# nackdai/aten

Measured on AMD Instinct MI355X. Metric: Mrays/sec (W*H*spp/1e6/s, reference definition), Sponza 1080p 1spp 5-bounce, higher is better.
Workload: dtype f32; 1 GPU; sponza_lod 1920x1080 1spp 5-bounce GGX+IBL, reference-built sponza_lod.sbvh (stand-in for missing sponza.obj); width=1920, height=1080, spp=1, max_depth=5, rr_depth=3, frames_in_flight=4, triangles=12852, bvh_nodes=38000, anyhit_twins=1, planar_area_lights=0

## Files before the change

### aten_amd/_hostlib.py

```python
import ctypes as C
import os

from . import build

_lib = None

ATNS_ABI_VERSION = 2

ORDER_AS_SPLIT, ORDER_AREA, ORDER_AREA_SMALL, ORDER_COUNT, ORDER_COUNT_SMALL, ORDER_NEAR_POINT = range(6)


class BvhOptions(C.Structure):
    _fields_ = [("spatial_splits", C.c_int32), ("spatial_alpha", C.c_float), ("object_bins", C.c_int32),
                ("spatial_bins", C.c_int32), ("sweep_below", C.c_int32), ("child_order", C.c_int32),
                ("max_refs_factor", C.c_float), ("order_point", C.c_float * 3),
                ("order_point_given", C.c_int32), ("reinsert_iterations", C.c_int32), ("reinsert_batch", C.c_float)]


class BvhStats(C.Structure):
    _fields_ = [("n_nodes", C.c_uint32), ("n_leaves", C.c_uint32), ("n_spatial_splits", C.c_uint32), ("n_reinsertions", C.c_uint32),
                ("sah_cost", C.c_float)]


def default_bvh_options(**kw):
# ... 32 lines not shown
                                            C.POINTER(BvhStats)]
        lib.atns_optimize_nodes.restype = C.c_int
        lib.atns_anyhit_twin.argtypes = [C.c_void_p, C.c_uint32, C.POINTER(C.c_void_p), C.POINTER(C.c_double), C.POINTER(C.c_double)]
        lib.atns_anyhit_twin.restype = C.c_int
        lib.atns_build_blas.argtypes = [C.c_void_p, C.c_void_p, C.c_void_p, C.c_uint32,
                                        C.POINTER(C.c_void_p), C.POINTER(C.c_uint32),
                                        C.POINTER(C.c_float), C.POINTER(C.c_float)]
        lib.atns_build_blas.restype = C.c_int
        lib.atns_build_tlas.argtypes = [C.c_void_p, C.c_void_p, C.c_void_p, C.c_void_p, C.c_uint32,
                                        C.POINTER(C.c_void_p), C.POINTER(C.c_uint32)]
        lib.atns_build_tlas.restype = C.c_int
        lib.atns_free.argtypes = [C.c_void_p]
        lib.atns_free.restype = None
        lib.atns_validate_nodes.argtypes = [C.c_void_p, C.c_uint32]
        lib.atns_validate_nodes.restype = C.c_int64
        lib.atns_create_camera.argtypes = [C.c_void_p, C.POINTER(C.c_float), C.POINTER(C.c_float), C.POINTER(C.c_float),
                                           C.c_float, C.c_float, C.c_float, C.c_int32, C.c_int32]
        lib.atns_create_camera.restype = C.c_int
        _lib = lib
    return _lib
```

### aten_amd/_lib.py

```python
import ctypes as C
import os

from . import build

_lib = None

K_NAMES = ["gen_path", "trace_closest", "shade", "trace_shadow", "accumulate_sample", "gather",
           "svgf_prepare", "svgf_temporal", "svgf_variance", "svgf_atrous", "trace_fused"]

SYMBOLS = [
    "atn_create", "atn_destroy", "atn_last_error", "atn_upload_scene", "atn_update_camera", "atn_update_tlas",
    "atn_init_sampler", "atn_set_random", "atn_set_screen_shard", "atn_render", "atn_reset", "atn_set_path_batches",
    "atn_set_frames_in_flight", "atn_bank_streams", "atn_side_stream", "atn_mgpu_set_frames_in_flight", "atn_set_sampling_options", "atn_sample_texture",
    "atn_svgf_render", "atn_svgf_set_motion_depth", "atn_svgf_reset", "atn_svgf_set_atrous_iterations",
    "atn_svgf_download", "atn_svgf_output_device", "atn_svgf_set_dilate_temporal_weight", "atn_svgf_denoise", "atn_svgf_upload",
    "atn_restir_set_options", "atn_restir_render", "atn_restir_set_motion_depth", "atn_restir_reset", "atn_restir_capture",
    "atn_restir_download", "atn_npr_render", "atn_npr_reset", "atn_npr_capture", "atn_npr_download",
    "atn_volume_render", "atn_volume_reset", "atn_volume_capture", "atn_volume_download", "atn_volume_phase_table",
    "atn_film_device", "atn_tile_device", "atn_tile_slots", "atn_anyhit_twins", "atn_planar_area_lights", "atn_stream", "atn_synchronize",
    "atn_assemble_tiles", "atn_assemble_tiles_on", "atn_download_film", "atn_upload_film", "atn_get_stats", "atn_get_kernel_times",
    "atn_reset_kernel_times", "atn_generate_paths", "atn_trace_closest", "atn_cmj_samples", "atn_cmj_batch", "atn_ray_offset", "atn_get_random", "atn_random_count",
    "atn_material_table", "atn_material_eval", "atn_compact", "atn_compact2", "atn_sizeof_scene_desc", "atn_sizeof_destination",
    "atn_abi_version", "atn_build_id",
    "atn_download_path_cost", "atn_update_geometry", "atn_scene_device_arrays", "atn_lbvh_rebuild_list", "atn_lbvh_build",
    "atn_mgpu_update_geometry", "atn_mgpu_lbvh_rebuild_list",
    "atn_skin_create", "atn_skin_update", "atn_skin_compute", "atn_lbvh_rebuild_list_skinned", "atn_skin_download",
    "atn_skin_download_list", "atn_skin_destroy",
    "atn_mgpu_create", "atn_mgpu_destroy", "atn_mgpu_last_error", "atn_mgpu_shard_count", "atn_mgpu_shard_device",
    "atn_mgpu_upload_scene", "atn_mgpu_update_tlas", "atn_mgpu_update_camera", "atn_mgpu_init_sampler",
    "atn_mgpu_set_random", "atn_mgpu_render", "atn_mgpu_reset", "atn_mgpu_synchronize", "atn_mgpu_film_device",
    "atn_mgpu_download_film",
    "atn_set_regeneration", "atn_get_regeneration", "atn_render_burst", "atn_regen_stage_counts",
    "atn_mgpu_set_regeneration", "atn_mgpu_render_burst", "atn_set_upload_options", "atn_libm_probe", "atn_set_shade_math",
]
# ... 72 lines not shown
        l.atn_npr_download.argtypes = [vp, C.c_int32, vp]
        l.atn_volume_render.argtypes = [vp, vp, vp]
        l.atn_volume_reset.argtypes = [vp]
        l.atn_volume_capture.argtypes = [vp, C.c_int32]
        l.atn_volume_download.argtypes = [vp, C.c_int32, vp]
        l.atn_volume_phase_table.argtypes = [vp, C.c_float, C.c_uint32, vp, vp, vp, vp, vp, vp]
        l.atn_svgf_set_dilate_temporal_weight.argtypes = [vp, C.c_int32]
        l.atn_svgf_denoise.argtypes = [vp, vp, C.c_int32, vp, vp]
        l.atn_svgf_upload.argtypes = [vp, C.c_int32, C.c_int32, C.c_int32, vp]
        l.atn_svgf_output_device.argtypes = [vp]
        l.atn_svgf_output_device.restype = vp
        l.atn_film_device.argtypes = [vp]; l.atn_film_device.restype = vp
        l.atn_tile_device.argtypes = [vp]; l.atn_tile_device.restype = vp
        l.atn_tile_slots.argtypes = [vp]; l.atn_tile_slots.restype = C.c_uint32
        l.atn_anyhit_twins.argtypes = [vp]; l.atn_anyhit_twins.restype = C.c_uint32
        l.atn_planar_area_lights.argtypes = [vp]; l.atn_planar_area_lights.restype = C.c_uint32
        l.atn_stream.argtypes = [vp]; l.atn_stream.restype = vp
        l.atn_side_stream.argtypes = [vp]; l.atn_side_stream.restype = vp
        l.atn_synchronize.argtypes = [vp]
        l.atn_assemble_tiles.argtypes = [vp, vp, C.c_int32, vp]
        l.atn_assemble_tiles_on.argtypes = [vp, vp, C.c_int32, vp, vp]
        l.atn_download_film.argtypes = [vp, vp]
        l.atn_upload_film.argtypes = [vp, C.c_int32, C.c_int32, vp]
        l.atn_get_stats.argtypes = [vp, vp]
        l.atn_get_kernel_times.argtypes = [vp, vp, vp]
        l.atn_reset_kernel_times.argtypes = [vp]
        l.atn_generate_paths.argtypes = [vp, C.c_int32, C.c_int32, C.c_int32, C.c_uint32, vp]
        l.atn_trace_closest.argtypes = [vp, vp, C.c_uint32, C.c_float, C.c_float, vp, vp]
        l.atn_cmj_samples.argtypes = [vp, C.c_uint32, C.c_uint32, C.c_uint32, C.c_int32, vp]
        l.atn_cmj_batch.argtypes = [vp, C.c_uint32, vp, vp, vp, C.c_int32, vp]
# ... 29 lines not shown
```

### aten_amd/csrc/aten_amd.hip

```cpp
#include <hip/hip_runtime.h>

#include <algorithm>
#include <cstdio>
#include <cstdlib>
#include <chrono>
#include <cstring>
#include <memory>
#include <random>
#include <string>
#include <vector>

#include "../../include/aten_amd.h"
#include "device/kernels.hpp"
#include "device/launch.hpp"
#include "device/svgf.hpp"
#include "device/restir.hpp"
#include "device/npr.hpp"
#include "device/volume.hpp"
#include "device/lbvh.hpp"
#include "device/skinning.hpp"
#include "host/scene_upload.hpp"
#include "host/ibl_precompute.hpp"

namespace atn {
// ... 74 lines not shown

    DevBuf<float4> nodes, vtx_pos, vtx_nml, matrices, texels, carpaint, shade_tris;
    DevBuf<atn_triangle_param> tris;
    DevBuf<atn_object_param> objects;
    DevBuf<DevMaterial> materials;
    DevBuf<atn_light_param> lights;
    DevBuf<float4> light_plane;
    DevBuf<DevTexture> textures;
    DevBuf<atn_toon_param> toon;
    DevBuf<atn_light_param> npr_lights;
    DevBuf<float> screen_shadow;
    DevBuf<uint32_t> texels8;
    DevScene scene{};
    bool has_scene = false, has_camera = false;
    std::vector<int32_t> list_root_link;
    uint32_t n_planar_lights = 0;
    struct PlanarCert {
        int32_t inst_obj = -1, mesh_obj = -1, mtx_id = -1;
        atn_object_param inst{}, mesh{};
        atn_mat4 l2w{}, w2l{};
        uint32_t tri_first = 0, tri_count = 0, vtx_lo = 0, vtx_hi = 0;
    };
    std::vector<PlanarCert> planar_certs;
    void collect_planar_certs(const atn_scene_desc* s, const std::vector<atn_light_param>& lights)
    {
        planar_certs.clear();
        for (size_t i = 0; i < lights.size() && i < s->n_lights; i++) {
            if (!lights[i]._pad) continue;
            PlanarCert c;
            c.inst_obj = s->lights[i].arealight_objid;
// ... 529 lines not shown
        { const int vrc = vol_decode(s, img); if (vrc) return vrc; }
        env_host.clear(); env_w = env_h = 0; ibl_tables_ready = false;
        {
            const int32_t ei = s->config.bg.envmap_tex_idx;
            if (ei >= 0 && (uint32_t)ei < s->n_textures && s->config.bg.enable_env_map) {
                const atn_texture_desc& t = s->textures[ei];
                env_host.assign(t.texels, t.texels + (size_t)t.width * t.height);
                env_w = t.width; env_h = t.height; env_multiplyer = s->config.bg.multiplyer;
            }
        }
        {
            int orc = apply_sampling_options();
            if (orc) return orc;
        }
        list_root_link = img.list_root_link; list_twin_delta = img.list_twin_delta; tlas_refs = img.tlas_refs;
        list_base = img.list_root; list_bytes = img.list_bytes; list_tri_leaves = img.list_tri_leaves; list_inner = img.list_inner;
        n_scene_tris = s->n_triangles; n_scene_vtx = s->n_vertices; n_scene_mtrls = s->n_materials;
        top_base = img.list_root[0];
        n_bottom_nodes = img.n_nodes - s->bvh_lists[0].count;
        n_host_matrices = s->n_matrices;
        host_matrices.assign(s->matrices, s->matrices + s->n_matrices);
        tree_is_deep = img.n_nodes >= kRefillMinNodes;
        return ATN_OK;
    }

    int apply_sampling_options()
    {
        scene.tex_bilinear = opt_tex_bilinear;
        scene.ibl_importance = 0;
        scene.ibl_cdf_v = nullptr; scene.ibl_cdf_u = nullptr; scene.ibl_w = 0; scene.ibl_h = 0;
// ... 232 lines not shown
        if ((uint64_t)tri_offset + n > n_scene_tris) return fail(ATN_ERR_INVALID_ARG, "triangle range outside the uploaded scene");
        if (list_tri_leaves[list] != n || list_inner[list] != n - 1 || list_bytes[list] != (n - 1) * kInnerBytes + n * kTriLeafBytes)
            return fail(ATN_ERR_UNSUPPORTED, "the list was not uploaded as a binary tree with one leaf per triangle of this range");
        ATN_HIP(hipSetDevice(device));
        const int32_t twin_word = list < list_twin_delta.size() ? list_twin_delta[list] : 0;
        const uint32_t twin_delta = (uint32_t)(twin_word & ~15), twin_dirs = twin_word == 0 ? 0u : ((twin_word & 1) ? 8u : 1u);
        if (twin_word != 0 && twin_delta != list_bytes[list]) return fail(ATN_ERR_UNSUPPORTED, "the list's twins do not lie at the list's own size apart");
        { int r = begin_scene_update(64); if (r) return r; }
        if (!box_dev) { int r = repack_shade_tris(tri_offset, n); if (r) return r; }
        { int r = lbvh_enqueue(tris.p + tri_offset, n, (int32_t)tri_offset, bmin, bmax, vtx_pos.p, 0, list_base[list], upd, box_dev); if (r) return r; }
        const uint32_t nn = 2 * n - 1;
        hipLaunchKernelGGL(k_lbvh_emit, dim3((nn + 255) / 256), dim3(256), 0, upd, n, (const atn_bvh_node*)lb.ref_nodes.p, (const uint32_t*)lb.offs.p,
                           (const atn_triangle_param*)tris.p, (const float4*)vtx_pos.p, nodes.p);
        ATN_HIP(hipGetLastError());
        log_range(SB_NODES, list_base[list], list_bytes[list]);
        if (twin_dirs) {
            if (lb.flips.n < n) ATN_HIP(lb.flips.resize(n));
            LbvhTopo t{ lb.left.p, lb.right.p, lb.parent.p, lb.first.p, lb.last.p };
            hipLaunchKernelGGL(k_lbvh_twin_flips, dim3((n + 255) / 256), dim3(256), 0, upd, n, t, (const atn_bvh_node*)lb.ref_nodes.p, twin_dirs, lb.flips.p);
            hipLaunchKernelGGL(k_lbvh_twin_emit, dim3((nn + 255) / 256, twin_dirs), dim3(256), 0, upd, n, t, (const atn_bvh_node*)lb.ref_nodes.p,
                               (const uint32_t*)lb.offs.p, (const uint8_t*)lb.flips.p, twin_delta, (const atn_triangle_param*)tris.p, (const float4*)vtx_pos.p, nodes.p);
            ATN_HIP(hipGetLastError());
            log_range(SB_NODES, list_base[list] + twin_delta, (size_t)twin_dirs * twin_delta);
        }
        { int r = end_scene_update(); if (r) return r; }
        if (sync) ATN_HIP(hipStreamSynchronize(upd));
        return ATN_OK;
    }

    struct Skin {
// ... 288 lines not shown
    {
        uint32_t b = (n + 255u) / 256u;
        if (b == 0) b = 1;
        return b < cap_blocks ? b : cap_blocks;
    }

    bool tree_is_deep = false;
    static constexpr size_t kRefillMinNodes = 2048;
    static constexpr uint32_t kRefillMinPaths = 400u * 1000u;
    bool refill_walk(bool frame) const
    {
        if (env_flavour >= 0) return env_flavour == 1;
        return tree_is_deep && (!frame || n_slots >= kRefillMinPaths);
    }

    uint32_t lds_scene_bytes() const
    {
        const uint64_t b = (uint64_t)scene.node_bytes + (uint64_t)scene.mtx_quads * 16u;
        return (env_lds_nodes && b <= kLdsNodesMaxBytes) ? (uint32_t)b : 0u;
    }

    uint32_t trace_grid(uint32_t n_jobs, bool refill) const
    {
        if (refill) {
            const uint32_t waves_per_block = (uint32_t)kTraceBlock / 64u;
            uint32_t blocks = ((n_jobs + atn::kFetchChunk - 1u) / atn::kFetchChunk + waves_per_block - 1u) / waves_per_block;
            if (blocks < 1u) blocks = 1u;
            const uint32_t cap = (frames_in_flight > 1 ? 256u * 18u : 256u * 32u) / waves_per_block;
            return blocks < cap ? blocks : cap;
        }
// ... 94 lines not shown
        for (int k = 0; k < nb; k++) {
            const uint32_t begin = (uint32_t)k * per;
            const uint32_t end = begin + per < n_slots ? begin + per : n_slots;
            if (begin >= end) continue;
            hipStream_t st = nb > 1 ? bstream[k] : stream;
            if (nb > 1) ATN_HIP(hipStreamWaitEvent(st, ev_fork, 0));
            PathBuffers pb = buffers(count, k, begin);
            fp.slot_begin = (int32_t)begin; fp.slot_end = (int32_t)end;
            const uint32_t n = end - begin;
            const PassPlan plan = plan_pass(SVGF ? PassKind::Svgf : PassKind::Serial, n);
            fp.chunk_items = plan.shade_items;
            const uint32_t g_slots = grid_for(n), g_all = (n + 255u) / 256u;
            for (int32_t s = 0; s < d->sample; s++) {
                fp.sample = s;
                if (s > 0) ATN_HIP(hipMemsetAsync(pb.q_count, 0, (size_t)4 * counters_depth * 4, st));
                prof_begin(prof, ATN_K_GEN, st);
                hipLaunchKernelGGL(k_gen_path, dim3(g_slots), dim3(256), 0, st, pb, fp, camera, (const uint32_t*)seeds.p);
                prof_end(prof);
                if (count || !fuse_traces) {
                    for (int32_t b = 0; b < d->maxDepth; b++) {
                        prof_begin(prof, ATN_K_TRACE_CLOSEST, st);
                        launch_trace<false>(plan, pb, count, b, st);
                        prof_end(prof);
                        prof_begin(prof, ATN_K_SHADE, st);
                        launch_shade<SVGF>(plan, st, pb, fp, b, sv);
                        prof_end(prof);
                        prof_begin(prof, ATN_K_TRACE_SHADOW, st);
                        launch_trace<true>(plan, pb, count, b, st);
                        prof_end(prof);
                    }
                }
                else {
                    for (int32_t b = 0; b <= d->maxDepth; b++) {
                        const TraceLaunch tl = trace_launch(plan, b);
                        prof_begin(prof, tl.prof_kind, st);
                        launch_trace_fused<false>(tl, st, pb, scene, b - 1, b < d->maxDepth ? b : -1, b);
                        prof_end(prof);
                        if (b < d->maxDepth) {
                            prof_begin(prof, ATN_K_SHADE, st);
                            launch_shade<SVGF>(plan, st, pb, fp, b, sv);
                            prof_end(prof);
                        }
                    }
                }
                if (SVGF || d->sample > 1) {
                    prof_begin(prof, ATN_K_ACCUM, st);
                    if (SVGF) hipLaunchKernelGGL(k_svgf_sample_end, dim3(g_all), dim3(256), 0, st, pb, fp, sf);
                    else hipLaunchKernelGGL(k_accumulate_sample, dim3(g_all), dim3(256), 0, st, pb, fp);
                    prof_end(prof);
                }
            }
            if (nb > 1) {
// ... 1399 lines not shown
    if (which == 9) { r.sv_motion_set = true; r.sv_motion_count = (size_t)width * height; }
    return ATN_OK;
}
void* atn_svgf_output_device(atn_ctx* ctx) { return ctx ? (void*)ctx->r.sv_out.p : nullptr; }

void* atn_film_device(atn_ctx* ctx) { return ctx ? (void*)ctx->r.film.p : nullptr; }
void* atn_tile_device(atn_ctx* ctx) { return ctx ? (void*)ctx->r.tile_out.p : nullptr; }
uint32_t atn_tile_slots(atn_ctx* ctx) { return ctx ? ctx->r.n_slots : 0; }
uint32_t atn_planar_area_lights(atn_ctx* ctx) { return (ctx && ctx->r.scene.planar_lights) ? ctx->r.n_planar_lights : 0u; }
uint32_t atn_anyhit_twins(atn_ctx* ctx)
{
    uint32_t n = 0;
    if (ctx) for (const int32_t d : ctx->r.list_twin_delta) n += d != 0 ? 1u : 0u;
    return n;
}
void* atn_stream(atn_ctx* ctx) { return ctx ? (void*)ctx->r.stream : nullptr; }
void* atn_side_stream(atn_ctx* ctx)
{
    if (!ctx) return nullptr;
    try { if (ctx->r.quiesce() != ATN_OK) return nullptr; return (void*)ctx->r.get_side_stream(); } catch (...) { return nullptr; }
}

int atn_synchronize(atn_ctx* ctx)
{
    CTX_QUIET_OR_FAIL(ctx);
    C_HIP(ctx->r, hipStreamSynchronize(ctx->r.stream));
    return ATN_OK;
}

int atn_assemble_tiles(atn_ctx* ctx, const void* gathered_dev, int32_t world, void* film_dev_out)
// ... 429 lines not shown
```

### aten_amd/csrc/device/kernels.hpp

```cpp
#pragma once
#include "shading.hpp"
#include "toon.hpp"

#if defined(ATN_REGEN_TU) || defined(ATN_TEMPLATES_ONLY)
#define ATN_MAIN_TU 0
#else
#define ATN_MAIN_TU 1
#endif
#ifdef ATN_REGEN_TU
#define ATN_REGEN_KERNELS 1
#else
#define ATN_REGEN_KERNELS 0
#endif

namespace atn {

constexpr uint32_t F_TERMINATED = 1u, F_SINGULAR = 2u, F_HIT = 4u;
constexpr uint32_t kShadowSlotMask = (1u << 26) - 1u;
constexpr uint32_t kShadowStencilFlag = 0x40000000u;
constexpr uint32_t F_LAST_SPECULAR = 8u;

constexpr uint32_t F_PENDING = 16u;
constexpr uint32_t kRegenFlagMask = 31u;
constexpr uint32_t kRegenBounceShift = 5u, kRegenBounceMask = 255u;
// ... 114 lines not shown

ATN_DEV void pinhole_sample(const atn_camera_param& cam, float s, float t, f3& org, f3& dir)
{
    s = 2.0F * s - 1.0F;
    t = 2.0F * t - 1.0F;
    const f3 cu = mk3(cam.u[0], cam.u[1], cam.u[2]), cv = mk3(cam.v[0], cam.v[1], cam.v[2]);
    const f3 center = mk3(cam.center[0], cam.center[1], cam.center[2]);
    const f3 origin = mk3(cam.origin[0], cam.origin[1], cam.origin[2]);
    f3 pos_on_lens = s * cu + t * cv;
    pos_on_lens = pos_on_lens + center;
    dir = normalize(pos_on_lens - origin);
    org = origin;
}

#if ATN_MAIN_TU
__global__ void __launch_bounds__(256) k_gen_path(PathBuffers pb, FrameParams fp, atn_camera_param cam,
                                                   const uint32_t* __restrict__ seeds)
{
    __shared__ BlockAppendShared sh;
    const uint32_t n = (uint32_t)fp.slot_end;
    for (uint32_t chunk = (uint32_t)fp.slot_begin + blockIdx.x * kChunk; chunk < n; chunk += gridDim.x * kChunk) {
        uint32_t flags = 0;
#pragma unroll 1
        for (int k = 0; k < kChunkItems; k++) {
            const uint32_t slot = chunk + (uint32_t)k * 256u + threadIdx.x;
            int32_t ix = 0, iy = 0;
            bool valid = slot < n && slot_to_pixel(fp, slot, ix, iy);
            if (valid && fp.sample > 0) valid = pb.done[slot] == 0;
            if (!valid) continue;
            const uint32_t idx = (uint32_t)(iy * fp.width + ix);
            const uint32_t rnd = seeds[idx % fp.n_seeds];
            const uint32_t fs = fp.frame + (uint32_t)fp.sample;
            const uint32_t scramble = rnd * 0x1fe3434fu * ((fs + 133u * rnd) / 256u);
            Cmj smp; smp.idx = fs % 256u; smp.dim = 0; smp.scramble = scramble;
            const float r1 = cmj_next(smp);
            const float r2 = cmj_next(smp);
            const float s = ((float)ix + r1) / (float)cam.width;
            const float t = ((float)iy + r2) / (float)cam.height;
            f3 org, dir;
            pinhole_sample(cam, s, t, org, dir);
            pb.ray_o[slot] = make_float4(org.x, org.y, org.z, 1.0F);
            pb.ray_d[slot] = make_float4(dir.x, dir.y, dir.z, __uint_as_float(0u));
            pb.thr[slot] = make_float4(1.0F, 1.0F, 1.0F, __uint_as_float(smp.dim));
            pb.contrib[slot] = make_float4(0.0F, 0.0F, 0.0F, 0.0F);
            if (fp.sample == 0) { pb.accum[slot] = make_float4(0, 0, 0, 0); pb.done[slot] = 0; }
            flags |= 1u << k;
        }
        block_append2(sh, pb.queue[0], &pb.q_count[0], flags, (uint32_t*)nullptr, (uint32_t*)nullptr, 0u,
                      [&](int k) { return chunk + (uint32_t)k * 256u + threadIdx.x; });
    }
}

#endif

struct RegenState { float4 o, d, t; };
ATN_DEV void regen_item(const PathBuffers& pb, const FrameParams& fp, uint32_t item, uint32_t& frame_k, uint32_t& pixel_slot)
{
    uint32_t j;
    udivmod(item, fp.n_valid, fp.n_valid_rcp, frame_k, j);
    pixel_slot = pb.valid_list[j];
}
// ... 185 lines not shown
};

template <bool COUNT, bool REFILL>
__global__ void __launch_bounds__(kTraceBlock > 256 ? kTraceBlock : 256) k_trace_closest(PathBuffers pb, DevScene sc, int32_t bounce)
{
    const uint32_t count = pb.q_count[bounce];
    const ClosestJob job{ pb, pb.queue[bounce & 1], kEps };
    TravCounters tc{};
    trace_dispatch<COUNT, REFILL>(sc, count, &pb.fetch_closest[bounce], job, &tc);
    if (COUNT) {
        if (blockIdx.x == 0 && threadIdx.x == 0) atomicAdd(&pb.stats[0], (unsigned long long)count);
        wave_add_stat(&pb.stats[3], tc.nodes);
        wave_add_stat(&pb.stats[4], tc.tris);
    }
}

struct SvgfShade {
    float4* nd;
    float4* am;
    float4* primary;
    float w2c3[4];
};

#ifdef ATN_SHADE_WPE
#define ATN_SHADE_ATTR __attribute__((amdgpu_waves_per_eu(ATN_SHADE_WPE, ATN_SHADE_WPE)))
#else
#define ATN_SHADE_ATTR
#endif
#ifndef ATN_SHADE_PARTITION
#define ATN_SHADE_PARTITION 1
// ... 883 lines not shown
```

### aten_amd/csrc/device/launch.hpp

```cpp
#pragma once
#include <type_traits>
#include "kernels.hpp"

namespace atn {

template <class F>
void with_flags(F&& f) { f(); }
template <class F, class... B>
void with_flags(F&& f, bool flag, B... rest)
{
    if (flag) with_flags([&](auto... x) { f(std::true_type{}, x...); }, rest...);
    else with_flags([&](auto... x) { f(std::false_type{}, x...); }, rest...);
}

template <int MS, int WAVES>
struct ShadeFlavour { static constexpr int ms = MS, waves = WAVES; };
template <class F>
void with_shade_flavour(int material_set, int waves, F&& f)
{
    switch (material_set) {
    case kMsCore: if (waves == 5) f(ShadeFlavour<kMsCore, 5>{}); else f(ShadeFlavour<kMsCore, 4>{}); break;
    case kMsDisney: if (waves == 5) f(ShadeFlavour<kMsDisney, 5>{}); else f(ShadeFlavour<kMsDisney, 4>{}); break;
    case kMsAnalytic: if (waves == 5) f(ShadeFlavour<kMsAnalytic, 5>{}); else f(ShadeFlavour<kMsAnalytic, 4>{}); break;
    case kMsCarPaint: f(ShadeFlavour<kMsCarPaint, 0>{}); break;
// ... 27 lines not shown
    const bool refill = p.refill && stage != 0;
    const bool closest = p.kind != PassKind::Regen && stage == 0 && p.lds_bytes == 0u;
    return TraceLaunch{ closest, refill, p.lds_bytes != 0u, refill ? p.fused_grid : p.fused_grid * (256u / p.block),
                        refill ? (uint32_t)kTraceBlock : p.block, p.lds_bytes, p.refill && stage == 0 ? ATN_K_TRACE_CLOSEST : ATN_K_TRACE_FUSED };
}

template <bool REGEN>
void launch_trace_fused(const TraceLaunch& l, hipStream_t st, const PathBuffers& pb, const DevScene& sc, int32_t bs, int32_t bc, int32_t launch)
{
    const dim3 g(l.grid), t(l.block);
    if constexpr (!REGEN) if (l.closest) { hipLaunchKernelGGL((k_trace_closest<false, false>), g, t, l.lds_bytes, st, pb, sc, bc); return; }
    with_flags([&](auto refill, auto alpha, auto lds) {
        hipLaunchKernelGGL((k_trace_fused<decltype(refill)::value, decltype(alpha)::value, decltype(lds)::value, REGEN>), g, t, l.lds_bytes, st, pb, sc, bs, bc, launch);
    }, l.refill, sc.any_alpha != 0, l.lds);
}

void regen_launch_begin(uint32_t grid, hipStream_t st, const PathBuffers& pb, const FrameParams& fp, const atn_camera_param& cam);
void regen_launch_trace(const TraceLaunch& l, hipStream_t st, const PathBuffers& pb, const DevScene& sc, int32_t bs, int32_t bc, int32_t launch);
void regen_launch_shade(int material_set, int waves, uint32_t grid, hipStream_t st, const PathBuffers& pb, const DevScene& sc, const FrameParams& fp,
                        const atn_camera_param& cam, int32_t stage, const RegenOut& ro);
void regen_launch_compact(uint32_t grid, hipStream_t st, const PathBuffers& pb, int32_t stage, uint32_t chunk_size, uint32_t* group_counts_next, uint32_t n_groups);
void regen_launch_flush(uint32_t grid, hipStream_t st, const PathBuffers& pb, const FrameParams& fp, const RegenOut& ro);
void regen_launch_end(uint32_t grid, hipStream_t st, const PathBuffers& pb, const FrameParams& fp, const RegenOut& ro);

void relaxed_launch_shade(int material_set, int waves, uint32_t grid, hipStream_t st, const PathBuffers& pb, const DevScene& sc, const FrameParams& fp,
                          const atn_camera_param& cam, int32_t bounce);

struct RestirArgs;
void restir_launch_shade(int material_set, uint32_t grid, hipStream_t st, const PathBuffers& pb, const DevScene& sc, const FrameParams& fp,
                         const atn_camera_param& cam, const RestirArgs& ra);
// ... 63 lines not shown
```

### aten_amd/csrc/device/traverse.hpp

```cpp
#pragma once
#include "scene_dev.hpp"

namespace atn {

struct Hit {
    float t;
    int32_t objid;
    int32_t tri;
    float a, b;
    int32_t meshid;
};

struct TravCounters { uint32_t nodes, tris, ray_nodes, ray_tris; };

struct RaySlab { f3 org, dir, invdir, oxinvdir; bool finite; };

ATN_DEV bool is_finite3(const f3& v)
{
    return (fabsf(v.x) <= kInf) && (fabsf(v.y) <= kInf) && (fabsf(v.z) <= kInf);
}

ATN_DEV void slab_setup(RaySlab& s, const f3& org, const f3& dir)
{
    s.org = org; s.dir = dir;
// ... 497 lines not shown
                if (w.node == kLinkEnd) {
                    const uint32_t k = bits_below_lane(m_idle);
                    if (k < avail) walk_start<LDSN, COUNT>(w, sc, stage[c_next + k][0], stage[c_next + k][1], stage_stop[c_next + k], cnt);
                }
                c_next += n_idle < avail ? n_idle : avail;
                all_finite = __all(w.node == kLinkEnd || w.ray.finite) != 0;
            }
            else if (n_idle == 64u) {
                break;
            }
        }
        walk_iteration<COUNT, kInnerBurst, Job, LDSN, ATN_DEFER_FINISH != 0>(w, all_finite, sc, nb, t_min, job, cnt, iter++);
    }
}

}
```

### aten_amd/csrc/host/bvh_builder.cpp

```cpp
#include "../../../include/aten_amd_scene.h"
#include "anyhit_twin.hpp"

#include <algorithm>
#include <cmath>
#include <cstdlib>
#include <cstring>
#include <limits>
#include <new>
#include <vector>

namespace {

constexpr float kInf = std::numeric_limits<float>::max();

struct Box {
    float mn[3], mx[3];
    void reset()
    {
        for (int k = 0; k < 3; k++) { mn[k] = kInf; mx[k] = -kInf; }
    }
    void grow(const Box& b)
    {
        for (int k = 0; k < 3; k++) { mn[k] = std::min(mn[k], b.mn[k]); mx[k] = std::max(mx[k], b.mx[k]); }
    }
// ... 827 lines not shown
    try {
        atn::AnyhitTwin tw;
        if (!atn::make_anyhit_twin(nodes, count, tw)) return -4;
        atn_bvh_node* o = (atn_bvh_node*)std::malloc(sizeof(atn_bvh_node) * tw.nodes.size());
        if (!o) return -3;
        std::memcpy(o, tw.nodes.data(), sizeof(atn_bvh_node) * tw.nodes.size());
        *out_nodes = o;
        if (out_cost_as_given) *out_cost_as_given = tw.cost_as_given;
        if (out_cost_twin) *out_cost_twin = tw.cost_twin;
        return 0;
    }
    catch (const std::bad_alloc&) { return -3; }
    catch (...) { return -5; }
}

void atns_free(void* p) { std::free(p); }

int64_t atns_validate_nodes(const atn_bvh_node* nodes, uint32_t count)
{
    if (!nodes) return -1;
    int64_t leaves = 0;
    for (uint32_t i = 0; i < count; i++) {
        const int32_t h = (int32_t)nodes[i].hit, m = (int32_t)nodes[i].miss;
        if (h < -1 || h >= (int32_t)count || m < -1 || m >= (int32_t)count) return -2;
    }
    int32_t id = 0; uint32_t steps = 0;
    while (id >= 0) {
        if (++steps > count) return -3;
        if (nodes[id].f0 >= 0 || nodes[id].f1 >= 0) leaves++;
        id = (int32_t)nodes[id].hit;
// ... 6 lines not shown
```

### aten_amd/csrc/host/scene_upload.hpp

```cpp
#pragma once
#include <cmath>
#include <cstring>
#include <string>
#include <vector>

#include "../device/scene_dev.hpp"
#include "anyhit_twin.hpp"

namespace atn {

struct HostSceneImage {
    std::vector<float4> nodes;
    uint64_t n_nodes = 0;
    std::vector<uint32_t> list_root;
    std::vector<int32_t> list_root_link;
    std::vector<uint32_t> list_bytes;
    std::vector<int32_t> list_twin_delta;
    struct TlasRef { uint32_t offset, list; };
    std::vector<TlasRef> tlas_refs;
    std::vector<uint32_t> list_tri_leaves, list_inner;
    std::vector<atn_triangle_param> tris;
    std::vector<float4> vtx_pos, vtx_nml;
    std::vector<atn_object_param> objects;
    std::vector<float4> matrices;
    std::vector<DevMaterial> materials;
    std::vector<float4> carpaint;
    std::vector<atn_toon_param> toon;
    std::vector<atn_light_param> npr_lights;
    std::vector<float> screen_shadow;
    std::vector<atn_light_param> lights;
    std::vector<float4> light_plane;
    std::vector<float4> texels;
    std::vector<uint32_t> texels8;
    std::vector<DevTexture> textures;
    DevScene params{};
// ... 312 lines not shown
        bool ok = true;
        for (uint32_t g = 0; g < n_dir && ok; g++) {
            if (n_dir > 1) {
                const int sg[3] = { (g & 1u) ? 1 : -1, (g & 2u) ? 1 : -1, (g & 4u) ? 1 : -1 };
                ok = make_anyhit_twin(s->bvh_lists[k].nodes, s->bvh_lists[k].count, tw, sg);
            }
            std::string twin_err;
            ok = ok && analyse_list(twin_lay[k][g], tw.nodes.data(), (uint32_t)tw.nodes.size(), false, twin_err);
            twin[k][g].swap(tw.nodes);
        }
        if (!ok) { twin[k].clear(); twin_lay[k].clear(); }
    }
    uint64_t off = 0;
    img.list_root.assign(nl, 0);
    img.list_bytes.assign(nl, 0); img.list_tri_leaves.assign(nl, 0); img.list_inner.assign(nl, 0); img.list_twin_delta.assign(nl, 0);
    for (uint32_t kk = 1; kk <= nl; kk++) {
        const uint32_t k = kk % nl;
        img.list_root[k] = (uint32_t)off;
        for (uint32_t j = 0; j < lay[k].order.size(); j++) {
            if (lay[k].kind[j] == KIND_TRI) img.list_tri_leaves[k]++;
            else if (lay[k].kind[j] == KIND_INNER) img.list_inner[k]++;
        }
        assign_offsets(lay[k], off, k == 0 ? 0 : node_layout_top_levels);
        if (off >= (1ull << 31)) { err = "too many BVH nodes for 31-bit byte-offset links"; return false; }
        img.list_bytes[k] = (uint32_t)(off - img.list_root[k]);
        if (!twin[k].empty()) {
            if (twin_lay[k][0].kind[0] != lay[k].kind[0] || off + (uint64_t)img.list_bytes[k] * twin[k].size() >= (1ull << 31)) { twin[k].clear(); continue; }
            img.list_twin_delta[k] = (int32_t)(off - img.list_root[k]) | (twin[k].size() > 1 ? 1 : 0);
            for (size_t g = 0; g < twin[k].size(); g++)
                assign_offsets(twin_lay[k][g], off, node_layout_top_levels);
// ... 185 lines not shown
```

### aten_amd/renderer.py

```python
import ctypes as C

import numpy as np

from . import layout as L
from ._lib import Destination, K_NAMES, lib


class AtenAmdError(RuntimeError):
    pass


class PathTracing:
    def __init__(self, device=0):
        self._l = lib()
        self._ctx = C.c_void_p()
        rc = self._l.atn_create(C.byref(self._ctx), device)
        if rc != 0:
            raise AtenAmdError("atn_create failed (%d): no usable HIP device; libaten_amd has no CPU fallback" % rc)
        if self._l.atn_sizeof_scene_desc() != C.sizeof(L.SceneDesc):
            raise AtenAmdError("atn_scene_desc ABI mismatch")
        if self._l.atn_sizeof_destination() != C.sizeof(Destination):
            raise AtenAmdError("atn_destination ABI mismatch")
        self.width = self.height = 0
        self._skin_sizes = {}
# ... 211 lines not shown
        return out

    def upload_film(self, film):
        film = np.ascontiguousarray(film, np.float32)
        h, w = film.shape[:2]
        self._check(self._l.atn_upload_film(self._ctx, w, h, film.ctypes.data))
        self.width, self.height = w, h

    def path_cost(self):
        out = np.zeros((self.height, self.width, 2), np.uint32)
        self._check(self._l.atn_download_path_cost(self._ctx, out.ctypes.data))
        return out

    def anyhit_twins(self):
        return int(self._l.atn_anyhit_twins(self._ctx))

    def planar_area_lights(self):
        return int(self._l.atn_planar_area_lights(self._ctx))

    def stats(self):
        s = np.zeros(8, np.uint64)
        self._check(self._l.atn_get_stats(self._ctx, s.ctypes.data))
        return dict(closest_rays=int(s[0]), shadow_rays=int(s[1]), hits=int(s[2]),
                    closest_nodes=int(s[3]), closest_tris=int(s[4]), shadow_nodes=int(s[5]), shadow_tris=int(s[6]))

    SVGF_BUFFERS = dict(normal_depth=0, albedo_meshid=1, color_variance=2, moment_temporalweight=3,
                        prev_normal_depth=4, prev_albedo_meshid=5, prev_color_variance=6, prev_moment_temporalweight=7,
                        temporary_color=8, motion_depth=9, primary_position=10, atrous0=11, atrous1=12, output=13,
                        contribs=14)

# ... 389 lines not shown
```

### include/aten_amd.h

```cpp
#ifndef ATEN_AMD_H_
#define ATEN_AMD_H_

#include "aten_layout.h"

#ifdef __cplusplus
extern "C" {
#endif

typedef struct atn_ctx atn_ctx;

typedef enum atn_status {
    ATN_OK = 0,
    ATN_ERR_INVALID_ARG = -1,
    ATN_ERR_NO_DEVICE = -2,
    ATN_ERR_HIP = -3,
    ATN_ERR_NO_SCENE = -4,
    ATN_ERR_UNSUPPORTED = -5,
    ATN_ERR_OUT_OF_MEMORY = -6
} atn_status;

typedef struct atn_destination {
    int32_t width;
    int32_t height;
    int32_t maxDepth;
// ... 50 lines not shown

int atn_render(atn_ctx* ctx, const atn_destination* dst, atn_vec4* out_host);

int atn_set_regeneration(atn_ctx* ctx, int32_t mode);
int32_t atn_get_regeneration(atn_ctx* ctx);
int atn_render_burst(atn_ctx* ctx, const atn_destination* dst, int32_t n_frames, atn_vec4* out_host);
int atn_regen_stage_counts(atn_ctx* ctx, uint32_t* closest, uint32_t* shadow, uint32_t capacity, uint32_t* n_stages);

int atn_set_shade_math(atn_ctx* ctx, int32_t mode);

int atn_reset(atn_ctx* ctx);

void* atn_film_device(atn_ctx* ctx);
void* atn_tile_device(atn_ctx* ctx);
uint32_t atn_anyhit_twins(atn_ctx* ctx);
uint32_t atn_planar_area_lights(atn_ctx* ctx);
uint32_t atn_tile_slots(atn_ctx* ctx);
void* atn_stream(atn_ctx* ctx);
int atn_synchronize(atn_ctx* ctx);

int atn_assemble_tiles(atn_ctx* ctx, const void* gathered_dev, int32_t world, void* film_dev_out);
int atn_assemble_tiles_on(atn_ctx* ctx, const void* gathered_dev, int32_t world, void* film_dev_out, void* hip_stream);
int atn_download_film(atn_ctx* ctx, atn_vec4* out_host);
int atn_upload_film(atn_ctx* ctx, int32_t width, int32_t height, const atn_vec4* film_host);

int atn_get_stats(atn_ctx* ctx, uint64_t out[8]);
int atn_download_path_cost(atn_ctx* ctx, uint32_t* out_host);

enum { ATN_K_GEN = 0, ATN_K_TRACE_CLOSEST = 1, ATN_K_SHADE = 2, ATN_K_TRACE_SHADOW = 3,
       ATN_K_ACCUM = 4, ATN_K_GATHER = 5,
// ... 99 lines not shown
```

### include/aten_amd_scene.h

```cpp
#ifndef ATEN_AMD_SCENE_H_
#define ATEN_AMD_SCENE_H_

#include "aten_layout.h"

#ifdef __cplusplus
extern "C" {
#endif

#define ATNS_ABI_VERSION 2u
uint32_t atns_abi_version(void);

int atns_build_blas(const atn_vec4* vtx_pos, const atn_triangle_param* tris,
                    const uint32_t* tri_ids, uint32_t n_tris,
                    atn_bvh_node** out_nodes, uint32_t* out_count,
                    float out_bbox_min[3], float out_bbox_max[3]);

enum {
    ATNS_ORDER_AS_SPLIT = 0,
    ATNS_ORDER_AREA = 1,
    ATNS_ORDER_AREA_SMALL = 2,
    ATNS_ORDER_COUNT = 3,
    ATNS_ORDER_COUNT_SMALL = 4,
    ATNS_ORDER_NEAR_POINT = 5
};
// ... 12 lines not shown
} atns_bvh_options;
typedef struct atns_bvh_stats {
    uint32_t n_nodes, n_leaves, n_spatial_splits, n_reinsertions;
    float sah_cost;
} atns_bvh_stats;
void atns_bvh_default_options(atns_bvh_options* out);
int atns_build_blas_opt(const atn_vec4* vtx_pos, const atn_triangle_param* tris,
                        const uint32_t* tri_ids, uint32_t n_tris, const atns_bvh_options* options,
                        atn_bvh_node** out_nodes, uint32_t* out_count,
                        float out_bbox_min[3], float out_bbox_max[3], atns_bvh_stats* out_stats);

int atns_optimize_nodes(const atn_bvh_node* nodes, uint32_t count, const atns_bvh_options* options,
                        atn_bvh_node** out_nodes, uint32_t* out_count, atns_bvh_stats* out_stats);

int atns_anyhit_twin(const atn_bvh_node* nodes, uint32_t count, atn_bvh_node** out_nodes, double* out_cost_as_given, double* out_cost_twin);

int atns_build_tlas(const float* boxes, const int32_t* object_ids, const int32_t* blas_list_ids,
                    const int32_t* mesh_ids, uint32_t n,
                    atn_bvh_node** out_nodes, uint32_t* out_count);

void atns_free(void* p);

int atns_create_camera(atn_camera_param* out, const float origin[3], const float lookat[3], const float up[3],
                       float vfov, float z_near, float z_far, int32_t width, int32_t height);

int64_t atns_validate_nodes(const atn_bvh_node* nodes, uint32_t count);

typedef struct atns_obj atns_obj;
typedef struct atns_obj_material_info {
    const char* name;
// ... 54 lines not shown
```

Before: 661.8 Mrays/s.

## Fuse primary ray generation into trace and add wave-coherent packet walk

Primary-ray generation is folded into a new k_trace_primary kernel that generates camera rays and traces them in the same pass, so the separate k_gen_path launch and its ray buffer round trip are dropped on the fused path. When the root BLAS is a threaded (stackless hit/miss link) list and the scene has no alpha, no LDS copy and no environment, primary rays use a packet walk. In that walk the whole wave follows one wave-uniform node pointer, read through scalar loads, and masks off lanes that missed a subtree. This exploits the coherence of camera rays, at the cost of extra node visits for divergent lanes and a host-side pass that checks each list for threading.

```diff
diff --git a/aten_amd/_hostlib.py b/aten_amd/_hostlib.py
--- a/aten_amd/_hostlib.py
+++ b/aten_amd/_hostlib.py
@@ -70,6 +70,8 @@
         lib.atns_free.restype = None
         lib.atns_validate_nodes.argtypes = [C.c_void_p, C.c_uint32]
         lib.atns_validate_nodes.restype = C.c_int64
+        lib.atns_list_is_threaded.argtypes = [C.c_void_p, C.c_uint32]
+        lib.atns_list_is_threaded.restype = C.c_int
         lib.atns_create_camera.argtypes = [C.c_void_p, C.POINTER(C.c_float), C.POINTER(C.c_float), C.POINTER(C.c_float),
                                            C.c_float, C.c_float, C.c_float, C.c_int32, C.c_int32]
         lib.atns_create_camera.restype = C.c_int
diff --git a/aten_amd/_lib.py b/aten_amd/_lib.py
--- a/aten_amd/_lib.py
+++ b/aten_amd/_lib.py
@@ -17,7 +17,7 @@
     "atn_restir_set_options", "atn_restir_render", "atn_restir_set_motion_depth", "atn_restir_reset", "atn_restir_capture",
     "atn_restir_download", "atn_npr_render", "atn_npr_reset", "atn_npr_capture", "atn_npr_download",
     "atn_volume_render", "atn_volume_reset", "atn_volume_capture", "atn_volume_download", "atn_volume_phase_table",
-    "atn_film_device", "atn_tile_device", "atn_tile_slots", "atn_anyhit_twins", "atn_planar_area_lights", "atn_stream", "atn_synchronize",
+    "atn_film_device", "atn_tile_device", "atn_tile_slots", "atn_anyhit_twins", "atn_primary_walk", "atn_planar_area_lights", "atn_stream", "atn_synchronize",
     "atn_assemble_tiles", "atn_assemble_tiles_on", "atn_download_film", "atn_upload_film", "atn_get_stats", "atn_get_kernel_times",
     "atn_reset_kernel_times", "atn_generate_paths", "atn_trace_closest", "atn_cmj_samples", "atn_cmj_batch", "atn_ray_offset", "atn_get_random", "atn_random_count",
     "atn_material_table", "atn_material_eval", "atn_compact", "atn_compact2", "atn_sizeof_scene_desc", "atn_sizeof_destination",
@@ -120,6 +120,7 @@
         l.atn_tile_device.argtypes = [vp]; l.atn_tile_device.restype = vp
         l.atn_tile_slots.argtypes = [vp]; l.atn_tile_slots.restype = C.c_uint32
         l.atn_anyhit_twins.argtypes = [vp]; l.atn_anyhit_twins.restype = C.c_uint32
+        l.atn_primary_walk.argtypes = [vp]; l.atn_primary_walk.restype = C.c_int
         l.atn_planar_area_lights.argtypes = [vp]; l.atn_planar_area_lights.restype = C.c_uint32
         l.atn_stream.argtypes = [vp]; l.atn_stream.restype = vp
         l.atn_side_stream.argtypes = [vp]; l.atn_side_stream.restype = vp
diff --git a/aten_amd/csrc/aten_amd.hip b/aten_amd/csrc/aten_amd.hip
--- a/aten_amd/csrc/aten_amd.hip
+++ b/aten_amd/csrc/aten_amd.hip
@@ -112,6 +112,7 @@
     DevScene scene{};
     bool has_scene = false, has_camera = false;
     std::vector<int32_t> list_root_link;
+    std::vector<uint8_t> list_threaded;
     uint32_t n_planar_lights = 0;
     struct PlanarCert {
         int32_t inst_obj = -1, mesh_obj = -1, mtx_id = -1;
@@ -671,6 +672,7 @@
             if (orc) return orc;
         }
         list_root_link = img.list_root_link; list_twin_delta = img.list_twin_delta; tlas_refs = img.tlas_refs;
+        list_threaded = img.list_threaded;
         list_base = img.list_root; list_bytes = img.list_bytes; list_tri_leaves = img.list_tri_leaves; list_inner = img.list_inner;
         n_scene_tris = s->n_triangles; n_scene_vtx = s->n_vertices; n_scene_mtrls = s->n_materials;
         top_base = img.list_root[0];
@@ -933,6 +935,7 @@
                            (const atn_triangle_param*)tris.p, (const float4*)vtx_pos.p, nodes.p);
         ATN_HIP(hipGetLastError());
         log_range(SB_NODES, list_base[list], list_bytes[list]);
+        if (list < list_threaded.size()) list_threaded[list] = 0;
         if (twin_dirs) {
             if (lb.flips.n < n) ATN_HIP(lb.flips.resize(n));
             LbvhTopo t{ lb.left.p, lb.right.p, lb.parent.p, lb.first.p, lb.last.p };
@@ -1251,6 +1254,15 @@
         return tree_is_deep && (!frame || n_slots >= kRefillMinPaths);
     }
 
+    int primary_walk() const
+    {
+        if (!has_scene) return kPrimaryPlain;
+        if (ATN_PRIMARY_PACKET && fuse_traces && env_flavour < 0 && scene.root_direct && lds_scene_bytes() == 0u && !scene.any_alpha)
+            for (size_t k = 1; k < list_root_link.size() && k < list_threaded.size(); k++)
+                if (list_root_link[k] == scene.root_blas && list_threaded[k]) return kPrimaryPacket;
+        return trace_launch(plan_pass(PassKind::Serial, n_slots ? n_slots : 1u), 0).refill ? kPrimaryRefill : kPrimaryPlain;
+    }
+
     uint32_t lds_scene_bytes() const
     {
         const uint64_t b = (uint64_t)scene.node_bytes + (uint64_t)scene.mtx_quads * 16u;
@@ -1375,9 +1387,12 @@
             for (int32_t s = 0; s < d->sample; s++) {
                 fp.sample = s;
                 if (s > 0) ATN_HIP(hipMemsetAsync(pb.q_count, 0, (size_t)4 * counters_depth * 4, st));
-                prof_begin(prof, ATN_K_GEN, st);
-                hipLaunchKernelGGL(k_gen_path, dim3(g_slots), dim3(256), 0, st, pb, fp, camera, (const uint32_t*)seeds.p);
-                prof_end(prof);
+                const bool fused_primary = !count && fuse_traces && env_flavour < 0;
+                if (!fused_primary) {
+                    prof_begin(prof, ATN_K_GEN, st);
+                    hipLaunchKernelGGL(k_gen_path, dim3(g_slots), dim3(256), 0, st, pb, fp, camera, (const uint32_t*)seeds.p);
+                    prof_end(prof);
+                }
                 if (count || !fuse_traces) {
                     for (int32_t b = 0; b < d->maxDepth; b++) {
                         prof_begin(prof, ATN_K_TRACE_CLOSEST, st);
@@ -1393,10 +1408,17 @@
                 }
                 else {
                     for (int32_t b = 0; b <= d->maxDepth; b++) {
-                        const TraceLaunch tl = trace_launch(plan, b);
-                        prof_begin(prof, tl.prof_kind, st);
-                        launch_trace_fused<false>(tl, st, pb, scene, b - 1, b < d->maxDepth ? b : -1, b);
-                        prof_end(prof);
+                        if (b == 0 && fused_primary) {
+                            prof_begin(prof, ATN_K_TRACE_CLOSEST, st);
+                            launch_trace_primary(primary_launch(plan, primary_walk() == kPrimaryPacket, n), st, pb, scene, fp, camera, (const uint32_t*)seeds.p);
+                            prof_end(prof);
+                        }
+                        else {
+                            const TraceLaunch tl = trace_launch(plan, b);
+                            prof_begin(prof, tl.prof_kind, st);
+                            launch_trace_fused<false>(tl, st, pb, scene, b - 1, b < d->maxDepth ? b : -1, b);
+                            prof_end(prof);
+                        }
                         if (b < d->maxDepth) {
                             prof_begin(prof, ATN_K_SHADE, st);
                             launch_shade<SVGF>(plan, st, pb, fp, b, sv);
@@ -2826,6 +2848,7 @@
     if (ctx) for (const int32_t d : ctx->r.list_twin_delta) n += d != 0 ? 1u : 0u;
     return n;
 }
+int atn_primary_walk(atn_ctx* ctx) { return ctx ? ctx->r.primary_walk() : 0; }
 void* atn_stream(atn_ctx* ctx) { return ctx ? (void*)ctx->r.stream : nullptr; }
 void* atn_side_stream(atn_ctx* ctx)
 {
diff --git a/aten_amd/csrc/device/kernels.hpp b/aten_amd/csrc/device/kernels.hpp
--- a/aten_amd/csrc/device/kernels.hpp
+++ b/aten_amd/csrc/device/kernels.hpp
@@ -152,6 +152,31 @@
 }
 
 #if ATN_MAIN_TU
+ATN_DEV bool gen_path_slot(const PathBuffers& pb, const FrameParams& fp, const atn_camera_param& cam, const uint32_t* __restrict__ seeds,
+                           uint32_t slot, uint32_t n, f3& org, f3& dir)
+{
+    int32_t ix = 0, iy = 0;
+    bool valid = slot < n && slot_to_pixel(fp, slot, ix, iy);
+    if (valid && fp.sample > 0) valid = pb.done[slot] == 0;
+    if (!valid) return false;
+    const uint32_t idx = (uint32_t)(iy * fp.width + ix);
+    const uint32_t rnd = seeds[idx % fp.n_seeds];
+    const uint32_t fs = fp.frame + (uint32_t)fp.sample;
+    const uint32_t scramble = rnd * 0x1fe3434fu * ((fs + 133u * rnd) / 256u);
+    Cmj smp; smp.idx = fs % 256u; smp.dim = 0; smp.scramble = scramble;
+    const float r1 = cmj_next(smp);
+    const float r2 = cmj_next(smp);
+    const float s = ((float)ix + r1) / (float)cam.width;
+    const float t = ((float)iy + r2) / (float)cam.height;
+    pinhole_sample(cam, s, t, org, dir);
+    pb.ray_o[slot] = make_float4(org.x, org.y, org.z, 1.0F);
+    pb.ray_d[slot] = make_float4(dir.x, dir.y, dir.z, __uint_as_float(0u));
+    pb.thr[slot] = make_float4(1.0F, 1.0F, 1.0F, __uint_as_float(smp.dim));
+    pb.contrib[slot] = make_float4(0.0F, 0.0F, 0.0F, 0.0F);
+    if (fp.sample == 0) { pb.accum[slot] = make_float4(0, 0, 0, 0); pb.done[slot] = 0; }
+    return true;
+}
+
 __global__ void __launch_bounds__(256) k_gen_path(PathBuffers pb, FrameParams fp, atn_camera_param cam,
                                                    const uint32_t* __restrict__ seeds)
 {
@@ -161,28 +186,8 @@
         uint32_t flags = 0;
 #pragma unroll 1
         for (int k = 0; k < kChunkItems; k++) {
-            const uint32_t slot = chunk + (uint32_t)k * 256u + threadIdx.x;
-            int32_t ix = 0, iy = 0;
-            bool valid = slot < n && slot_to_pixel(fp, slot, ix, iy);
-            if (valid && fp.sample > 0) valid = pb.done[slot] == 0;
-            if (!valid) continue;
-            const uint32_t idx = (uint32_t)(iy * fp.width + ix);
-            const uint32_t rnd = seeds[idx % fp.n_seeds];
-            const uint32_t fs = fp.frame + (uint32_t)fp.sample;
-            const uint32_t scramble = rnd * 0x1fe3434fu * ((fs + 133u * rnd) / 256u);
-            Cmj smp; smp.idx = fs % 256u; smp.dim = 0; smp.scramble = scramble;
-            const float r1 = cmj_next(smp);
-            const float r2 = cmj_next(smp);
-            const float s = ((float)ix + r1) / (float)cam.width;
-            const float t = ((float)iy + r2) / (float)cam.height;
             f3 org, dir;
-            pinhole_sample(cam, s, t, org, dir);
-            pb.ray_o[slot] = make_float4(org.x, org.y, org.z, 1.0F);
-            pb.ray_d[slot] = make_float4(dir.x, dir.y, dir.z, __uint_as_float(0u));
-            pb.thr[slot] = make_float4(1.0F, 1.0F, 1.0F, __uint_as_float(smp.dim));
-            pb.contrib[slot] = make_float4(0.0F, 0.0F, 0.0F, 0.0F);
-            if (fp.sample == 0) { pb.accum[slot] = make_float4(0, 0, 0, 0); pb.done[slot] = 0; }
-            flags |= 1u << k;
+            if (gen_path_slot(pb, fp, cam, seeds, chunk + (uint32_t)k * 256u + threadIdx.x, n, org, dir)) flags |= 1u << k;
         }
         block_append2(sh, pb.queue[0], &pb.q_count[0], flags, (uint32_t*)nullptr, (uint32_t*)nullptr, 0u,
                       [&](int k) { return chunk + (uint32_t)k * 256u + threadIdx.x; });
@@ -398,6 +403,55 @@
         wave_add_stat(&pb.stats[4], tc.tris);
     }
 }
+
+#if ATN_MAIN_TU
+struct PrimaryJob {
+    const PathBuffers& pb;
+    const FrameParams& fp;
+    const atn_camera_param& cam;
+    const uint32_t* __restrict__ seeds;
+    float t_min;
+    ATN_DEV bool fetch(uint32_t slot, float4& a, float4& b, float& stop_t) const
+    {
+        f3 org, dir;
+        if (!gen_path_slot(pb, fp, cam, seeds, slot, (uint32_t)fp.slot_end, org, dir)) return false;
+        stop_t = -kInf;
+        a = make_float4(org.x, org.y, org.z, kInf);
+        b = make_float4(dir.x, dir.y, dir.z, __uint_as_float(slot));
+        return true;
+    }
+    ATN_DEV bool finish(uint32_t slot, const Hit& h, bool, float4&, float4&, float&) const
+    {
+        pb.isect[slot] = make_float4(__int_as_float(h.objid), h.a, h.b, __int_as_float(h.tri));
+        return false;
+    }
+    ATN_DEV void cost(uint32_t, uint32_t, uint32_t) const {}
+};
+
+template <bool PACKET, bool LDSN>
+__global__ void __attribute__((amdgpu_waves_per_eu(PACKET ? 8 : 1, 8))) __launch_bounds__(256) k_trace_primary(PathBuffers pb, DevScene sc, FrameParams fp, atn_camera_param cam,
+                                                        const uint32_t* __restrict__ seeds)
+{
+    __shared__ BlockAppendShared sh;
+    const PrimaryJob job{ pb, fp, cam, seeds, kEps };
+    if constexpr (LDSN) lds_scene_copy(sc);
+    const uint32_t n = (uint32_t)fp.slot_end;
+    for (uint32_t chunk = (uint32_t)fp.slot_begin + blockIdx.x * kChunk; chunk < n; chunk += gridDim.x * kChunk) {
+        uint32_t flags = 0;
+#pragma unroll 1
+        for (int k = 0; k < kChunkItems; k++) {
+            float4 a = make_float4(0.0F, 0.0F, 0.0F, 0.0F), b = a;
+            float stop_t;
+            const bool valid = job.fetch(chunk + (uint32_t)k * 256u + threadIdx.x, a, b, stop_t);
+            if (valid) flags |= 1u << k;
+            if constexpr (PACKET) trace_packet(sc, job, valid, a, b);
+            else trace_tile<PrimaryJob, LDSN>(sc, job, valid, a, b);
+        }
+        block_append2(sh, pb.queue[0], &pb.q_count[0], flags, (uint32_t*)nullptr, (uint32_t*)nullptr, 0u,
+                      [&](int k) { return chunk + (uint32_t)k * 256u + threadIdx.x; });
+    }
+}
+#endif
 
 struct SvgfShade {
     float4* nd;
diff --git a/aten_amd/csrc/device/launch.hpp b/aten_amd/csrc/device/launch.hpp
--- a/aten_amd/csrc/device/launch.hpp
+++ b/aten_amd/csrc/device/launch.hpp
@@ -65,6 +65,32 @@
         hipLaunchKernelGGL((k_trace_fused<decltype(refill)::value, decltype(alpha)::value, decltype(lds)::value, REGEN>), g, t, l.lds_bytes, st, pb, sc, bs, bc, launch);
     }, l.refill, sc.any_alpha != 0, l.lds);
 }
+
+#ifndef ATN_PRIMARY_PACKET
+#define ATN_PRIMARY_PACKET 1
+#endif
+enum PrimaryWalk { kPrimaryPlain = 0, kPrimaryRefill = 1, kPrimaryPacket = 2 };
+struct PrimaryLaunch {
+    bool packet, lds;
+    uint32_t grid, lds_bytes;
+};
+inline PrimaryLaunch primary_launch(const PassPlan& p, bool packet, uint32_t n_slots)
+{
+    uint32_t grid = (n_slots + kChunk - 1u) / kChunk;
+    if (grid < 1u) grid = 1u;
+    if (grid > 256u * 16u) grid = 256u * 16u;
+    return PrimaryLaunch{ packet && p.lds_bytes == 0u, p.lds_bytes != 0u, grid, p.lds_bytes };
+}
+#if ATN_MAIN_TU
+inline void launch_trace_primary(const PrimaryLaunch& l, hipStream_t st, const PathBuffers& pb, const DevScene& sc, const FrameParams& fp,
+                                 const atn_camera_param& cam, const uint32_t* seeds)
+{
+    const dim3 g(l.grid), t(256);
+    if (l.packet) hipLaunchKernelGGL((k_trace_primary<true, false>), g, t, 0, st, pb, sc, fp, cam, seeds);
+    else if (l.lds) hipLaunchKernelGGL((k_trace_primary<false, true>), g, t, l.lds_bytes, st, pb, sc, fp, cam, seeds);
+    else hipLaunchKernelGGL((k_trace_primary<false, false>), g, t, 0, st, pb, sc, fp, cam, seeds);
+}
+#endif
 
 void regen_launch_begin(uint32_t grid, hipStream_t st, const PathBuffers& pb, const FrameParams& fp, const atn_camera_param& cam);
 void regen_launch_trace(const TraceLaunch& l, hipStream_t st, const PathBuffers& pb, const DevScene& sc, int32_t bs, int32_t bc, int32_t launch);
diff --git a/aten_amd/csrc/device/traverse.hpp b/aten_amd/csrc/device/traverse.hpp
--- a/aten_amd/csrc/device/traverse.hpp
+++ b/aten_amd/csrc/device/traverse.hpp
@@ -535,4 +535,78 @@
     }
 }
 
-}
+
+template <class Job, bool LDSN>
+ATN_DEV void trace_tile(const DevScene& sc, const Job& job, bool valid, const float4& a, const float4& b)
+{
+    const char* __restrict__ nb = reinterpret_cast<const char*>(sc.nodes);
+    const float t_min = sc.bvh_hit_min > 0 ? sc.bvh_hit_min : job.t_min;
+    Walk w;
+    walk_start<LDSN, false>(w, sc, a, b, -kInf);
+    if (!valid) w.node = kLinkEnd;
+    if constexpr (LDSN && kSimpleBurstLds > 0) {
+        w.pending = false;
+        bool all_finite = __all(w.node == kLinkEnd || w.ray.finite) != 0;
+        while (__any(w.node != kLinkEnd))
+            walk_iteration<false, kSimpleBurstLds, Job, true, true>(w, all_finite, sc, nb, t_min, job, nullptr);
+        (void)walk_finish<false, Job, true>(w, sc, job, nullptr);
+    }
+    else {
+        static_assert(!LDSN || kSimpleBurstLds > 0, "the per-ray walk reads global memory");
+        walk_run<false>(w, sc, nb, t_min, nullptr);
+        float4 ra, rb;
+        float rstop;
+        if (valid) (void)job.finish(w.payload, w.hit, w.hit.objid >= 0, ra, rb, rstop);
+    }
+}
+
+typedef float atn_v4f __attribute__((ext_vector_type(4)));
+typedef const __attribute__((address_space(4))) atn_v4f* atn_const_v4f_ptr;
+ATN_DEV float4 ld16_uniform(const char* base, uint32_t byte_off)
+{
+    const atn_v4f v = *(atn_const_v4f_ptr)(base + byte_off);
+    return make_float4(v.x, v.y, v.z, v.w);
+}
+
+constexpr int32_t kWaitNone = 4;
+template <class Job>
+ATN_DEV void trace_packet(const DevScene& sc, const Job& job, bool valid, const float4& a, const float4& b)
+{
+    const char* nb = reinterpret_cast<const char*>(sc.nodes);
+    const float t_min = sc.bvh_hit_min > 0 ? sc.bvh_hit_min : job.t_min;
+    Walk w;
+    walk_start<false, false>(w, sc, a, b, -kInf);
+    int32_t cur = __any(valid) ? __builtin_amdgcn_readfirstlane(sc.root_blas) : kLinkEnd;
+    int32_t wait = valid ? kWaitNone : kLinkEnd;
+    bool all_finite = __all(!valid || w.ray.finite) != 0;
+    while (cur != kLinkEnd) {
+        const bool part = wait == kWaitNone;
+        if (cur >= 0) {
+            const float4 q0 = ld16_uniform(nb, (uint32_t)cur), q1 = ld16_uniform(nb, (uint32_t)cur + 16u);
+            bool box = false;
+            if (part) {
+                box = all_finite ? slab_hit_fast(w.ray, mk3(q0), mk3(q1), t_min, w.t_max)
+                                 : slab_hit_exact(w.ray, mk3(q0), mk3(q1), t_min, w.t_max);
+                if (!box) wait = __float_as_int(q1.w);
+            }
+            cur = __any(box) ? __float_as_int(q0.w) : __float_as_int(q1.w);
+        }
+        else {
+            const uint32_t off = (uint32_t)cur & kLinkOffsetMask;
+            const float4 q0 = ld16_uniform(nb, off), q1 = ld16_uniform(nb, off + 16u), q2 = ld16_uniform(nb, off + 32u);
+            if (part) {
+                bool accept; float t;
+                (void)leaf_test(w.ray, q0, q1, q2, t_min, w.hit, w.t_max, w.objid, w.meshid, accept, t);
+            }
+            cur = __float_as_int(q1.w);
+        }
+        cur = __builtin_amdgcn_readfirstlane(cur);
+        if (wait == cur) wait = kWaitNone;
+        if (!all_finite) all_finite = __all(wait == kLinkEnd || w.ray.finite) != 0;
+    }
+    float4 ra, rb;
+    float rstop;
+    if (valid) (void)job.finish(w.payload, w.hit, w.hit.objid >= 0, ra, rb, rstop);
+}
+
+}
diff --git a/aten_amd/csrc/host/bvh_builder.cpp b/aten_amd/csrc/host/bvh_builder.cpp
--- a/aten_amd/csrc/host/bvh_builder.cpp
+++ b/aten_amd/csrc/host/bvh_builder.cpp
@@ -1,5 +1,6 @@
 #include "../../../include/aten_amd_scene.h"
 #include "anyhit_twin.hpp"
+#include "list_threading.hpp"
 
 #include <algorithm>
 #include <cmath>
@@ -865,6 +866,13 @@
     catch (...) { return -5; }
 }
 
+int atns_list_is_threaded(const atn_bvh_node* nodes, uint32_t count)
+{
+    if (!nodes || atns_validate_nodes(nodes, count) < 0) return -1;
+    try { return atn::list_is_threaded(nodes, count) ? 1 : 0; }
+    catch (...) { return -3; }
+}
+
 void atns_free(void* p) { std::free(p); }
 
 int64_t atns_validate_nodes(const atn_bvh_node* nodes, uint32_t count)
diff --git a/aten_amd/csrc/host/list_threading.hpp b/aten_amd/csrc/host/list_threading.hpp
--- /dev/null
+++ b/aten_amd/csrc/host/list_threading.hpp
@@ -0,0 +1,31 @@
+#pragma once
+#include <cstdint>
+#include <vector>
+
+#include "../../../include/aten_layout.h"
+
+namespace atn {
+
+inline bool list_is_threaded(const atn_bvh_node* src, uint32_t count)
+{
+    if (count == 0) return false;
+    auto link = [](float f) { const int32_t l = (int32_t)f; return l < 0 ? -1 : l; };
+    auto inner = [&](int32_t i) { return !(src[i].f0 >= 0 || src[i].f1 >= 0); };
+    if (link(src[0].miss) != -1) return false;
+    struct Frame { int32_t c, exit; };
+    std::vector<Frame> open;
+    std::vector<uint8_t> seen(count, 0);
+    if (inner(0)) open.push_back(Frame{ link(src[0].hit), -1 });
+    while (!open.empty()) {
+        const Frame f = open.back();
+        if (f.c == f.exit) { open.pop_back(); continue; }
+        if (f.c < 0 || (uint32_t)f.c >= count || seen[f.c]) return false;
+        seen[f.c] = 1;
+        const int32_t next = link(src[f.c].miss);
+        open.back().c = next;
+        if (inner(f.c)) open.push_back(Frame{ link(src[f.c].hit), next });
+    }
+    return true;
+}
+
+}
diff --git a/aten_amd/csrc/host/scene_upload.hpp b/aten_amd/csrc/host/scene_upload.hpp
--- a/aten_amd/csrc/host/scene_upload.hpp
+++ b/aten_amd/csrc/host/scene_upload.hpp
@@ -6,6 +6,7 @@
 
 #include "../device/scene_dev.hpp"
 #include "anyhit_twin.hpp"
+#include "list_threading.hpp"
 
 namespace atn {
 
@@ -19,6 +20,7 @@
     struct TlasRef { uint32_t offset, list; };
     std::vector<TlasRef> tlas_refs;
     std::vector<uint32_t> list_tri_leaves, list_inner;
+    std::vector<uint8_t> list_threaded;
     std::vector<atn_triangle_param> tris;
     std::vector<float4> vtx_pos, vtx_nml;
     std::vector<atn_object_param> objects;
@@ -361,6 +363,8 @@
     uint64_t off = 0;
     img.list_root.assign(nl, 0);
     img.list_bytes.assign(nl, 0); img.list_tri_leaves.assign(nl, 0); img.list_inner.assign(nl, 0); img.list_twin_delta.assign(nl, 0);
+    img.list_threaded.assign(nl, 0);
+    for (uint32_t k = 1; k < nl; k++) img.list_threaded[k] = list_is_threaded(s->bvh_lists[k].nodes, s->bvh_lists[k].count) ? 1 : 0;
     for (uint32_t kk = 1; kk <= nl; kk++) {
         const uint32_t k = kk % nl;
         img.list_root[k] = (uint32_t)off;
diff --git a/aten_amd/renderer.py b/aten_amd/renderer.py
--- a/aten_amd/renderer.py
+++ b/aten_amd/renderer.py
@@ -249,6 +249,9 @@
 
     def anyhit_twins(self):
         return int(self._l.atn_anyhit_twins(self._ctx))
+
+    def primary_walk(self):
+        return int(self._l.atn_primary_walk(self._ctx))
 
     def planar_area_lights(self):
         return int(self._l.atn_planar_area_lights(self._ctx))
diff --git a/include/aten_amd.h b/include/aten_amd.h
--- a/include/aten_amd.h
+++ b/include/aten_amd.h
@@ -88,6 +88,7 @@
 void* atn_film_device(atn_ctx* ctx);
 void* atn_tile_device(atn_ctx* ctx);
 uint32_t atn_anyhit_twins(atn_ctx* ctx);
+int atn_primary_walk(atn_ctx* ctx);
 uint32_t atn_planar_area_lights(atn_ctx* ctx);
 uint32_t atn_tile_slots(atn_ctx* ctx);
 void* atn_stream(atn_ctx* ctx);
diff --git a/include/aten_amd_scene.h b/include/aten_amd_scene.h
--- a/include/aten_amd_scene.h
+++ b/include/aten_amd_scene.h
@@ -50,6 +50,8 @@
                         atn_bvh_node** out_nodes, uint32_t* out_count, atns_bvh_stats* out_stats);
 
 int atns_anyhit_twin(const atn_bvh_node* nodes, uint32_t count, atn_bvh_node** out_nodes, double* out_cost_as_given, double* out_cost_twin);
+
+int atns_list_is_threaded(const atn_bvh_node* nodes, uint32_t count);
 
 int atns_build_tlas(const float* boxes, const int32_t* object_ids, const int32_t* blas_list_ids,
                     const int32_t* mesh_ids, uint32_t n,
```

Result: faster. 674.9 Mrays/s (median of 6 runs) (+2.0%).
